# xiph/LPCNet

Hardware: AMD Instinct MI355X
Metric: 16 kHz samples/sec & concurrent real-time streams, 1/2/4/8 MI355X (higher is better)
Workload: dtype f32; 1 GPU; 2048 concurrent streams (each with its own feature file) per GPU x 25 frames (4000 samples) per step, fp32 weights, register-resident block-sparse GRU-A, bit-exact (PARITY) arithmetic; eight streams per CU as two groups of four half a step apart (BASELINE config 2's 1024 streams fill half of these stream slots: `also.config2_1024_streams`); arithmetic=parity, gru_a_blocks=1382, gru_a_densities=0.05,0.05,0.2 (benchmark model), gru_a_items_per_lane=30, streams_per_gpu=2048, streams_per_workgroup=8

## Files before the change

lpcnet_amd/csrc/sample_kernel_x2.hip.h:

```cpp
#pragma once
#include "sample_kernel.hip.h"
#include "tree_stages.h"

namespace lpcn {

#define LPCN_X2_LW 4
#define LPCN_X2_TW 0
#define LPCN_X2_HG 10

struct LdsX2 {
    static constexpr int S = 4;
    static constexpr int HA_STRIDE = 16 * S;
    static constexpr int g_hA    = 0;
    static constexpr int g_hT    = g_hA + 96 * HA_STRIDE + 24 * 16;
    static constexpr int g_prec  = g_hT + NA * S * 4;
    static constexpr int g_hB    = g_prec + NA * S * 4;
    static constexpr int g_idx   = g_hB + S * NB * 4;
    static constexpr int g_thr   = g_idx + S * 16;
    static constexpr int g_mask  = g_thr + S * 32;
    static constexpr int g_lead  = g_mask + S * 64;
    static constexpr int g_flag  = g_lead + S * 32;
    static constexpr int g_condb = g_flag + 16;
    static constexpr int g_lpc   = g_condb + S * RB * 4;
    static constexpr int g_pcm   = g_lpc + S * 64;
    static constexpr int G_SZ    = g_pcm + S * 320;
    static constexpr int pre_ur  = 2 * G_SZ;
    static constexpr int inh     = pre_ur + 2 * NA * S * 4;
    static constexpr int abias   = inh + NA * S * 4;
    static constexpr int tansig  = abias + 2 * RA * 4;
    static constexpr int ulaw    = tansig + 816;
    static constexpr int logit   = ulaw + 1024;
    static constexpr int brec    = logit + 1024;
    static constexpr int bbias   = brec + NB * RB * 4;
    static constexpr int bstart  = bbias + 2 * RB * 4;
    static constexpr int bw      = bstart + 32;
    static constexpr int total(int nb_b) { return bw + (nb_b + 8) * 128; }
    __host__ __device__ static constexpr int ha_off(int p) { return p * HA_STRIDE + (p >> 2) * 16; }
};

typedef float tree_f4 __attribute__((ext_vector_type(4)));
struct TreeRow { tree_f4 w[NB / 4]; float bias, factor; };
template <int STAGE>
__device__ __forceinline__ TreeRow tree_row_load(const LPCN_GLOBAL float *fc_w, const LPCN_GLOBAL float *fc_b, const LPCN_GLOBAL float *fc_f, const int lane, const int prefix)
{
    const int node = lpcn_tree_node(STAGE, lpcn_tree_lane_local(STAGE, lane), prefix), chan = lane & 1;
    const auto *wp = (const LPCN_GLOBAL tree_f4 *)(fc_w + (node * 2 + chan) * NB);
    TreeRow r;
#pragma unroll
    for (int j = 0; j < NB / 4; ++j) r.w[j] = wp[j];
    r.bias = fc_b[chan * 256 + node];
    r.factor = fc_f[chan * 256 + node];
    return r;
}
template <int STAGE>
__device__ __forceinline__ int tree_stage_walk(const TreeRow &r, const float *h_s, const float *thr_s, const float *tansig, const int lane)
{
    const float4 *hp = (const float4 *)h_s;
    float sum = r.bias;
#pragma unroll
    for (int j = 0; j < NB / 4; ++j) {
        const float4 hv = hp[j];
        const tree_f4 wv = r.w[j];
        sum = sum + wv[0] * hv.x;
        sum = sum + wv[1] * hv.y;
        sum = sum + wv[2] * hv.z;
        sum = sum + wv[3] * hv.w;
    }
    const float v = r.factor * lpcn_tanh(sum, tansig);
    const float vo = __builtin_bit_cast(float, __builtin_amdgcn_mov_dpp(__builtin_bit_cast(int, v), 0xB1, 0xf, 0xf, true));
    const float lg = v + vo;
    const unsigned long long m = __ballot(thr_s[lpcn_tree_level(STAGE, lpcn_tree_lane_local(STAGE, lane))] < lg) & lpcn_tree_stage_mask(STAGE);
    return lpcn_tree_stage_walk(m, STAGE == 0 ? LPCN_TREE_TOP : LPCN_TREE_LEVELS - LPCN_TREE_TOP);
}

template <int NW>
__global__ __launch_bounds__(LPCN_WG_THREADS, 2) void sample_kernel_x2(const LpcnSampleArgs *__restrict__ Ap)
{
    using L = LdsX2;
    constexpr int S = 4;
    constexpr int LW = LPCN_X2_LW, TW = LPCN_X2_TW;
    extern __shared__ __attribute__((aligned(16))) unsigned char smem[];
    float *const sm_pre_ur = (float *)(smem + L::pre_ur);
    float *const sm_inh = (float *)(smem + L::inh);
    const float *const sm_abias = (const float *)(smem + L::abias);
    const float *const sm_tansig = (const float *)(smem + L::tansig);
    const float *const sm_ulaw = (const float *)(smem + L::ulaw);
    const float *const sm_logit = (const float *)(smem + L::logit);
    const float *const sm_brec = (const float *)(smem + L::brec);
    const float *const sm_bbias = (const float *)(smem + L::bbias);
    const int *const sm_bstart = (const int *)(smem + L::bstart);

    const int tid0 = threadIdx.x;
    const int n_streams = Ap->n_streams, n_frames = Ap->n_frames, preload = Ap->preload, frame_len = Ap->frame_len;
    const int s0 = blockIdx.x * 2 * S;
    auto stream_of = [&](int gs) __attribute__((always_inline)) { return (s0 + gs < n_streams) ? s0 + gs : n_streams - 1; };
    const int n_valid = (n_streams - s0 < 2 * S) ? n_streams - s0 : 2 * S;
    const size_t nf = (size_t)n_frames;
    auto *const states = as_global_rw(Ap->state);
    const LPCN_GLOBAL float *emb_nat_sig = as_global(Ap->emb_nat_sig), *emb_nat_pred = as_global(Ap->emb_nat_pred), *emb_nat_exc = as_global(Ap->emb_nat_exc);
    asm volatile("" : "+s"(emb_nat_sig), "+s"(emb_nat_pred), "+s"(emb_nat_exc));

    float4 w[NW];
    uint32_t offp[(NW + 1) / 2];
    int row_reg[3];
#define LPCN_ROW(k) (row_reg[k])
    {
        const int lane = tid0 & 63, wave = tid0 >> 6;
        const size_t base = (size_t)wave * NW * 64 + lane;
        const int lane_sel = (lane & 3) * 16;
        const auto *ab = as_global(Ap->a_blk);
        const auto *aw = (const LPCN_GLOBAL float *)as_global(Ap->a_w);
#pragma unroll
        for (int j = 0; j < NW; ++j) {
            const auto *v = aw + (base + (size_t)j * 64) * 4;
            w[j] = make_float4(v[0], v[1], v[2], v[3]);
        }
#pragma unroll
        for (int j = 0; j < NW; j += 2) {
            const int p0 = ab[base + (size_t)j * 64];
            const int p1 = (j + 1 < NW) ? ab[base + (size_t)(j + 1) * 64] : 0;
            offp[j >> 1] = (uint32_t)(L::ha_off(p0) + lane_sel) | ((uint32_t)(L::ha_off(p1) + lane_sel) << 16);
        }
        const auto *ar = as_global(Ap->a_row);
#pragma unroll
        for (int k = 0; k < 3; ++k) row_reg[k] = ar[(wave * 3 + k) * 64 + lane];
    }
    int b1 = __builtin_amdgcn_readfirstlane(as_global(Ap->a_bound)[(tid0 >> 6) * 4 + 1]);
    int b2 = __builtin_amdgcn_readfirstlane(as_global(Ap->a_bound)[(tid0 >> 6) * 4 + 2]);
    int b3 = __builtin_amdgcn_readfirstlane(as_global(Ap->a_bound)[(tid0 >> 6) * 4 + 3]);
    const bool allh0 = __builtin_amdgcn_readfirstlane(as_global(Ap->a_allh)[(tid0 >> 6) * 3]) != 0;
    const LPCN_GLOBAL float *fc_w_s = as_global(Ap->fc_w), *fc_b_s = as_global(Ap->fc_b), *fc_f_s = as_global(Ap->fc_f);
    asm volatile("" : "+s"(fc_w_s), "+s"(fc_b_s), "+s"(fc_f_s));
    const LPCN_GLOBAL float *cond_a_s = as_global(Ap->cond_a);
    asm volatile("" : "+s"(cond_a_s));
    const int has_slot = __builtin_amdgcn_readfirstlane((__ballot(row_reg[0] >= 0) != 0ull ? 1 : 0) | (__ballot(row_reg[1] >= 0) != 0ull ? 2 : 0) |
                                                        (__ballot(row_reg[2] >= 0) != 0ull ? 4 : 0));
    const bool has2 = (has_slot & 4) != 0;
    const int hl = __builtin_amdgcn_readfirstlane(as_global(Ap->a_head)[tid0 >> 6]);
    const bool early_wave = hl > 0;
    const bool plain_start = __builtin_amdgcn_readfirstlane(((early_wave || __ballot(row_reg[0] >= 2 * NA) == 0ull) && __ballot(row_reg[1] >= 2 * NA || row_reg[2] >= 2 * NA) == 0ull) ? 1 : 0) != 0;

    {
        const int tid = tid0;
        stage_tables<L>(smem, Ap, tid, NB * RB);
        stage_grub_weights(smem + L::bw, Ap, tid, true);
        for (int i = tid; i < 2 * S * NA; i += LPCN_WG_THREADS) {
            const int gs = i / NA, n = i % NA, g = gs >> 2, s = gs & 3;
            const float hv0 = states[stream_of(gs)].gru_a[n];
            unsigned char *gb = smem + g * L::G_SZ;
            ((float *)(gb + L::g_hT))[n * S + s] = hv0;
            *(float *)(gb + L::g_hA + L::ha_off(n >> 2) + s * 16 + (n & 3) * 4) = hv0;
        }
        for (int i = tid; i < 2 * S * NB; i += LPCN_WG_THREADS) {
            const int gs = i / NB, g = gs >> 2, s = gs & 3;
            ((float *)(smem + g * L::G_SZ + L::g_hB))[s * NB + i % NB] = states[stream_of(gs)].gru_b[i % NB];
        }
        if (tid < 2 * S) {
            const int g = tid >> 2, s = tid & 3;
            unsigned char *gb = smem + g * L::G_SZ;
            stage_leader_record({(float *)(gb + L::g_lead), (int *)(gb + L::g_idx), nullptr, nullptr}, s, &states[stream_of(tid)]);
        }
        if (tid < 2) { int *fl = (int *)(smem + tid * L::G_SZ + L::g_flag); fl[0] = 0; fl[1] = 0; }
    }
    __syncthreads();

    const bool is_lw = (tid0 >> 6) == LW;
    const bool is_tw_lane = tid0 >= 64 * TW && tid0 < 64 * TW + S;
#define LPCN_LROW ((tid0 & 63) >> 4)
#define LPCN_TAP (tid0 & 15)
    float histP = is_lw ? states[stream_of(S + LPCN_LROW)].last_sig[LPCN_TAP] : 0.f;
    float histQ = is_lw ? states[stream_of(LPCN_LROW)].last_sig[LPCN_TAP] : 0.f;
    bool liveP = false, liveQ = false;
    int live_maskP = 0, live_maskQ = 0;
    int seqP = 0, seqQ = 0;
    int smpP = 0, smpQ = 0, fP = 0, fQ = 0;
    float lpc_tap = 0.f, prod_old = 0.f;

    const int T = n_frames * frame_len;
#if LPCN_ENABLE_PROF
#ifndef LPCN_PROF_MASK
#define LPCN_PROF_MASK 0xFFF
#endif
    unsigned long long *const prof = Ap->prof;
    unsigned long long pt[12] = {0, 0, 0, 0, 0, 0, 0, 0, 0, 0, 0, 0}, tprev = 0;
    const bool profiling = prof != nullptr && blockIdx.x == 0;
#define LPCN_X2_PROF(slot) do { if (((LPCN_PROF_MASK >> (slot)) & 1) && profiling) { const unsigned long long now_ = __builtin_amdgcn_s_memtime(); pt[slot] += now_ - tprev; tprev = now_; } } while (0)
    if (profiling) tprev = __builtin_amdgcn_s_memtime();
#else
#define LPCN_X2_PROF(slot) do { } while (0)
#endif
    for (int h = -1; h <= 2 * T + 1; ++h) {
        const int p = h & 1, q = p ^ 1;
        unsigned char *const gp = smem + p * L::G_SZ, *const gq = smem + q * L::G_SZ;
        const bool p_active = h >= 0 && (h >> 1) < T;
        const bool p_prev = h >= 2;
        const bool q_chain = h >= 1 && ((h - 1) >> 1) < T;
        const bool q_heads = ((h + 1) >> 1) < T;
        const bool new_frame = p_active && smpP == 0;
        const bool more = p_active && smpP != 0;
        float *const hT_p = (float *)(gp + L::g_hT);
        float *const hB_q = (float *)(gq + L::g_hB);
        int *const idx_p = (int *)(gp + L::g_idx);
        float *const lpc_p = (float *)(gp + L::g_lpc);
        short *const pcm_p = (short *)(gp + L::g_pcm);
        const LeaderCells cells_p = {(float *)(gp + L::g_lead), idx_p, (float *)(gp + L::g_thr), pcm_p};
        const uint32_t flag_p = lds_addr(gp + L::g_flag);

        if (more) ++seqP;
        if (p_prev && is_lw) {
            __builtin_amdgcn_s_setprio(3);
            const int smp_done = smpP == 0 ? frame_len - 1 : smpP - 1;
            int t_ = tid0;
            LPCN_REMAT_V(t_);
            const int lrow = (t_ & 63) >> 4, tap = t_ & 15;
            float pcm, deemph;
            int exc;
            draw_sample_walked(cells_p, (const int *)(gp + L::g_mask) + lrow, sm_ulaw, lrow, tap, liveP, smp_done, preload, histP, pcm, deemph, exc);
            if (more) { open_sample<S>(cells_p, tid0, liveP, pcm, tap == 0 ? pcm * lpc_tap : prod_old, exc, false); lds_publish(flag_p, seqP); }
            __builtin_amdgcn_s_setprio(0);
            finish_sample(cells_p, lrow, tap, liveP, smp_done, preload, pcm, deemph);
        }
        if (more && is_tw_lane && liveP) { int t_ = tid0; LPCN_REMAT_V(t_); draw_thresholds(cells_p, sm_logit, t_ - 64 * TW); }

        if (new_frame) {
            int tid = tid0;
            LPCN_REMAT_V(tid);
            const bool lw_ = (tid >> 6) == LW, twl_ = tid >= 64 * TW && tid < 64 * TW + S;
            __syncthreads();
            if (fP > 0) {
                auto *out = as_global_rw(Ap->pcm);
                const size_t pstride = (size_t)Ap->pcm_stride;
                for (int i = tid; i < S * LPCN_FRAME_SIZE; i += LPCN_WG_THREADS) {
                    const int s = i / LPCN_FRAME_SIZE, k = i % LPCN_FRAME_SIZE;
                    if (S * p + s < n_valid && k < frame_len) out[(size_t)(s0 + S * p + s) * pstride + (size_t)(fP - 1) * LPCN_FRAME_SIZE + k] = pcm_p[i];
                }
            }
            __syncthreads();
            {
                const auto *cb = as_global(Ap->cond_b), *lp = as_global(Ap->lpc);
                float *const condb_p = (float *)(gp + L::g_condb);
                if (tid < S * RB) condb_p[tid] = cb[((size_t)stream_of(S * p + tid / RB) * nf + fP) * RB + tid % RB];
                if (tid >= 256 && tid < 256 + S * LPCN_LPC_ORDER) {
                    const int i = tid - 256;
                    lpc_p[i] = lp[((size_t)stream_of(S * p + i / LPCN_LPC_ORDER) * nf + fP) * LPCN_LPC_ORDER + i % LPCN_LPC_ORDER];
                }
                if (lw_ || twl_) {
                    const int lstream = stream_of(S * p + (lw_ ? (tid & 63) >> 4 : tid - 64 * TW));
                    liveP = stream_is_live(Ap, states, lstream, fP);
                }
                if (preload > 0 && tid < S) {
                    const auto *pin = as_global(Ap->pcm) + (size_t)stream_of(S * p + tid) * (size_t)Ap->pcm_stride + (size_t)fP * LPCN_FRAME_SIZE;
                    for (int i = 0; i < preload; ++i) pcm_p[tid * LPCN_FRAME_SIZE + i] = pin[i];
                }
            }
            __syncthreads();
            ++seqP;
            if (lw_) {
                open_sample<S>(cells_p, tid0, liveP, histP, histP * lpc_p[tid & 63], ((const int *)cells_p.lead)[((tid & 63) >> 4) * 8 + 2], true);
                lds_publish(flag_p, seqP);
            }
            if (twl_ && liveP) draw_thresholds(cells_p, sm_logit, tid - 64 * TW);
            __syncthreads();
            int lm = 0;
#pragma unroll
            for (int s = 0; s < S; ++s) lm |= (idx_p[S + s] ? 1 : 0) << s;
            live_maskP = __builtin_amdgcn_readfirstlane(lm);
        }

        LPCN_X2_PROF(0);
        float acc[S] = {};
        constexpr int PF = 2;
        float4 hq[PF + 1] = {};
        const unsigned char *hA_cur = gp + L::g_hA;
        auto fetch_h = [&](const int j) __attribute__((always_inline)) {
            uint32_t pk = offp[j >> 1];
            LPCN_REMAT_V(pk);
            const uint32_t off = (j & 1) ? (pk >> 16) : (pk & 0xFFFFu);
            hq[j % (PF + 1)] = *(const float4 *)(hA_cur + off);
        };
        typedef float negz_t __attribute__((ext_vector_type(4)));
        negz_t negz = {-0.f, -0.f, -0.f, -0.f};
        auto load_negz = [&]() __attribute__((always_inline)) { negz = (negz_t){-0.f, -0.f, -0.f, -0.f}; asm volatile("" : "+v"(negz)); };
        auto mac = [&](const int j) __attribute__((always_inline)) {
            typedef float f4 __attribute__((ext_vector_type(4)));
            typedef float f2 __attribute__((ext_vector_type(2)));
            const float4 hv = hq[j % (PF + 1)];
            const float hk[4] = {hv.x, hv.y, hv.z, hv.w};
            const float wk[4] = {w[j].x, w[j].y, w[j].z, w[j].w};
            f2 a01 = {acc[0], acc[1]}, a23 = {acc[2], acc[3]};
            f4 pv[4];
#pragma unroll
            for (int c = 0; c < 4; ++c) pv[c] = __builtin_amdgcn_mfma_f32_4x4x1f32(hk[c], wk[c], negz, 0, 0, 0);
            __builtin_amdgcn_sched_barrier(0);
#pragma unroll
            for (int c = 0; c < 4; ++c) {
                a01 = a01 + __builtin_shufflevector(pv[c], pv[c], 0, 1);
                a23 = a23 + __builtin_shufflevector(pv[c], pv[c], 2, 3);
            }
            acc[0] = a01[0]; acc[1] = a01[1]; acc[2] = a23[0]; acc[3] = a23[1];
        };
        auto pre_cell = [&](const int r, unsigned char *gb) __attribute__((always_inline)) -> float * {
            return (float *)(r < 2 * NA ? smem + L::pre_ur + r * (S * 4) : gb + L::g_prec + (r - 2 * NA) * (S * 4));
        };

        const int wave = __builtin_amdgcn_readfirstlane(tid0 >> 6);

        constexpr int J0 = NW - LPCN_EARLY_MAX < 0 ? 0 : NW - LPCN_EARLY_MAX;
        constexpr int JM = J0 + LPCN_X2_HG < NW ? J0 + LPCN_X2_HG : NW;
        const bool do_heads = early_wave && q_heads;
        int e0 = NW - hl;
        LPCN_REMAT_S(e0);
        auto head_step = [&](auto self, auto jc, auto jend_c) __attribute__((always_inline)) -> void {
            constexpr int j = decltype(jc)::value, je = decltype(jend_c)::value;
            if constexpr (j < je) {
                if constexpr (j + PF < NW) fetch_h(j + PF);
                if (j >= e0) { asm volatile(""); mac(j); }
                self(self, std::integral_constant<int, j + 1>{}, jend_c);
            }
        };
        const uint32_t p0cnt_p = flag_p + 4;
        constexpr int CW = LPCN_X2_CHAIN_WAVES, P0W = LPCN_X2_P0_FIRST, NP0 = LPCN_WAVES - P0W;
        static_assert(NP0 * 64 * 3 == 2 * NA && CW == S, "three rounds of the row waves' lanes cover GRU-A's update / reset rows");
        const bool p0_wave = p_active && wave >= P0W;
        uint32_t o_sig[S] = {}, o_pred[S] = {}, o_exc[S] = {}, o_cond[S] = {};
        constexpr int P0PERM = 0x3102;
        int i0 = 0;
        float ld[3][4 * S] = {};
        auto p0_open = [&]() __attribute__((always_inline)) {
            int gi[S];
            {
                typedef int i4 __attribute__((ext_vector_type(4)));
                i4 v;
                int f;
                const uint32_t idx_a = lds_addr(idx_p);
                do {
                    asm volatile("ds_read_b32 %0, %2\n\tds_read_b128 %1, %3\n\ts_waitcnt lgkmcnt(0)" : "=&v"(f), "=&v"(v) : "v"(flag_p), "v"(idx_a) : "memory");
                    f = __builtin_amdgcn_readfirstlane(f);
                } while (f != seqP);
#pragma unroll
                for (int s = 0; s < S; ++s) gi[s] = __builtin_amdgcn_readfirstlane(v[s]);
            }
#pragma unroll
            for (int s = 0; s < S; ++s) {
                o_sig[s] = (uint32_t)(gi[s] & 0xFF) * (uint32_t)(RA * 4);
                o_pred[s] = (uint32_t)((gi[s] >> 8) & 0xFF) * (uint32_t)(RA * 4);
                o_exc[s] = ((uint32_t)(gi[s] >> 16) & 0xFFu) * (uint32_t)(RA * 4);
                o_cond[s] = (uint32_t)(((size_t)stream_of(S * p + s) * nf + (size_t)fP) * RA * 4);
            }
            int t_ = tid0;
            LPCN_REMAT_V(t_);
            i0 = (((P0PERM >> (4 * ((t_ >> 6) & 3))) & 3) << 6) | (t_ & 63);
        };
        const bool fifth = ((P0PERM >> (4 * (wave & 3))) & 3) < 2;
        auto issue = [&](const int k, const int buf) __attribute__((always_inline)) {
            const uint32_t rb = (uint32_t)(i0 + 256 * k) * 4u;
#pragma unroll
            for (int s = 0; s < S; ++s) {
                ld[buf][4 * s + 0] = *(const LPCN_GLOBAL float *)((const LPCN_GLOBAL char *)cond_a_s + (o_cond[s] + rb));
                ld[buf][4 * s + 1] = *(const LPCN_GLOBAL float *)((const LPCN_GLOBAL char *)emb_nat_sig + (o_sig[s] + rb));
                ld[buf][4 * s + 2] = *(const LPCN_GLOBAL float *)((const LPCN_GLOBAL char *)emb_nat_pred + (o_pred[s] + rb));
                ld[buf][4 * s + 3] = *(const LPCN_GLOBAL float *)((const LPCN_GLOBAL char *)emb_nat_exc + (o_exc[s] + rb));
            }
        };
        auto reduce = [&](const int k, const int buf) __attribute__((always_inline)) {
            const int r = i0 + 256 * k;
            float g[S];
#pragma unroll
            for (int s = 0; s < S; ++s) g[s] = ((ld[buf][4 * s + 0] + ld[buf][4 * s + 1]) + ld[buf][4 * s + 2]) + ld[buf][4 * s + 3];
            if (k < 3) {
                const int n = r >= NA ? r - NA : r;
                const float2 bd = *(const float2 *)(sm_abias + 2 * r);
                const float4 hv = *(const float4 *)(hT_p + n * S);
                *(float4 *)(sm_pre_ur + r * S) = make_float4((bd.x + bd.y * hv.x) + g[0], (bd.x + bd.y * hv.y) + g[1], (bd.x + bd.y * hv.z) + g[2], (bd.x + bd.y * hv.w) + g[3]);
            } else {
                *(float4 *)(sm_inh + (r - 2 * NA) * S) = make_float4(g[0], g[1], g[2], g[3]);
            }
        };
        if (wave < CW) {
            if (q_chain) {
                __builtin_amdgcn_s_setprio(3);
                const int s = wave;
                int ln_ = tid0;
                LPCN_REMAT_V(ln_);
                ln_ &= 63;
                const int r = ln_ < RB ? ln_ : RB - 1;
                const int g6 = r >> 3, ri = r & 7;
                const float *const condb_q = (const float *)(gq + L::g_condb);
                float zrh = sm_bbias[r] + condb_q[s * RB + r];
                float rec = sm_bbias[RB + r];
#pragma unroll
                for (int j = 0; j < NB; ++j) rec = rec + sm_brec[j * RB + r] * hB_q[s * NB + j];
                uint32_t wp32 = lds_addr(smem + L::bw + (sm_bstart[g6] * 8 + ri) * 16 + ((LPCN_GRUB_SHIFT >> (4 * g6)) & 15) * 128);
                uint32_t hp32 = lds_addr(gq + L::g_hA + s * 16);
                asm volatile(
#include "grub_lds_loop_s4.inc"
                    : [z] "+v"(zrh), [wp] "+v"(wp32), [hp] "+v"(hp32) : : LPCN_GRUB_LDS_CLOBBERS);
                __builtin_amdgcn_s_setprio(0);
                LPCN_X2_PROF(1);
                const TreeRow top = tree_row_load<0>(fc_w_s, fc_b_s, fc_f_s, ln_, 0);
                const int ln = ln_ & 15;
                const float sg = lpcn_sigmoid(zrh + rec, sm_tansig);
                const float r_gate = __builtin_bit_cast(float, __builtin_amdgcn_ds_bpermute((16 + ln) << 2, __builtin_bit_cast(int, sg)));
                const float hc = lpcn_tanh(zrh + rec * r_gate, sm_tansig);
                const float hc_i = __builtin_bit_cast(float, __builtin_amdgcn_ds_bpermute((32 + ln) << 2, __builtin_bit_cast(int, hc)));
                if (ln_ < NB) {
                    const float hold = hB_q[s * NB + ln_];
                    const float hnew = sg * hold + (1.f - sg) * hc_i;
                    if ((live_maskQ >> s) & 1) hB_q[s * NB + ln_] = hnew;
                }
                LPCN_X2_PROF(2);
                const float *const thr_s = (const float *)(gq + L::g_thr) + s * 8;
                int val = tree_stage_walk<0>(top, hB_q + s * NB, thr_s, sm_tansig, ln_);
                const TreeRow sub = tree_row_load<1>(fc_w_s, fc_b_s, fc_f_s, ln_, val);
                val = (val << (LPCN_TREE_LEVELS - LPCN_TREE_TOP)) | tree_stage_walk<1>(sub, hB_q + s * NB, thr_s, sm_tansig, ln_);
                if (ln_ == 0) ((int *)(gq + L::g_mask))[s] = val;
                LPCN_X2_PROF(9);
            }
        } else {
            if (do_heads) {
                hA_cur = gq + L::g_hA;
                load_negz();
                {
                    int r = LPCN_ROW(0);
                    LPCN_REMAT_V(r);
                    r = r < 0 ? 0 : r;
                    const int n = r - 2 * NA;
                    const float bias = sm_abias[2 * r], diag = sm_abias[2 * r + 1];
                    const float *hT_q = (const float *)(gq + L::g_hT);
#pragma unroll
                    for (int s = 0; s < S; ++s) acc[s] = bias + diag * hT_q[n * S + s];
                }
#pragma unroll
                for (int j = 0; j < PF; ++j) if (J0 + j < NW) fetch_h(J0 + j);
                head_step(head_step, std::integral_constant<int, J0>{}, std::integral_constant<int, JM>{});
            }
            LPCN_X2_PROF(3);
            if (p0_wave) {
                p0_open();
                LPCN_X2_PROF(1);
                issue(0, 0); issue(1, 1); issue(2, 2);
                LPCN_X2_PROF(2);
                reduce(0, 0); reduce(1, 1); reduce(2, 2);
                lds_arrive(p0cnt_p);
                issue(3, 0);
                if (fifth) issue(4, 1);
            }
            LPCN_X2_PROF(4);
            if (do_heads) {
                head_step(head_step, std::integral_constant<int, JM>{}, std::integral_constant<int, NW>{});
                int r = LPCN_ROW(0);
                LPCN_REMAT_V(r);
                if (r >= 0) {
                    float *c = pre_cell(r, gq);
#pragma unroll
                    for (int s = 0; s < S; ++s) c[s] = acc[s];
                }
            }
            if (p0_wave) { reduce(3, 0); if (fifth) reduce(4, 1); }
            LPCN_X2_PROF(3);
        }

        if (p_active) {
            hA_cur = gp + L::g_hA;
            load_negz();
            lds_poll_until<false>(p0cnt_p, seqP * NP0);
            LPCN_X2_PROF(11);
            if (plain_start) {
                int r = LPCN_ROW(0);
                LPCN_REMAT_V(r);
                r = r < 0 ? 0 : r;
                const float *c = pre_cell(r, gp);
#pragma unroll
                for (int s = 0; s < S; ++s) acc[s] = c[s];
            } else {
#pragma unroll
            for (int k = 0; k < 3; ++k) {
                int r = LPCN_ROW(k);
                LPCN_REMAT_V(r);
                const bool live_row = r >= 0;
                r = r < 0 ? 0 : r;
                const bool candidate = r >= 2 * NA;
                const int n = candidate ? r - 2 * NA : 0;
                const float bias = sm_abias[2 * r], diag = sm_abias[2 * r + 1];
                float *c = pre_cell(r, gp);
                const bool parked = k == 0 && early_wave;
#pragma unroll
                for (int s = 0; s < S; ++s) {
                    const float bv = bias + diag * hT_p[n * S + s];
                    if (k == 0) acc[s] = (candidate && !parked) ? bv : c[s];
                    else if (candidate && live_row) c[s] = bv;
                }
            }
            }
            auto row_swap = [&](const int k_done, const int k_next) __attribute__((always_inline)) {
                int r = LPCN_ROW(k_done), r2 = LPCN_ROW(k_next);
                LPCN_REMAT_V(r);
                LPCN_REMAT_V(r2);
                if (r >= 0) {
                    float *c = pre_cell(r, gp);
#pragma unroll
                    for (int s = 0; s < S; ++s) c[s] = acc[s];
                }
                r2 = r2 < 0 ? 0 : r2;
                const float *c2 = pre_cell(r2, gp);
#pragma unroll
                for (int s = 0; s < S; ++s) acc[s] = c2[s];
            };
            auto row_store = [&](const int k) __attribute__((always_inline)) {
                int r = LPCN_ROW(k);
                LPCN_REMAT_V(r);
                if (r >= 0) {
                    float *c = pre_cell(r, gp);
#pragma unroll
                    for (int s = 0; s < S; ++s) c[s] = acc[s];
                }
            };
            const int jend = b3;
            LPCN_X2_PROF(4);
#pragma unroll
            for (int j = 0; j < PF && j < NW; ++j) fetch_h(j);
            LPCN_REMAT_S(b1);
            LPCN_REMAT_S(b2);
            LPCN_REMAT_S(b3);
            int nextb = b1;
            LPCN_REMAT_S(nextb);
            auto item = [&](const int j) __attribute__((always_inline)) -> bool {
                if (__builtin_expect(j >= jend, 0)) return false;
                if (j + PF < NW) fetch_h(j + PF);
                if (__builtin_expect(j == nextb, 0)) {
                    if (j == b1) row_swap(0, 1);
                    if (j == b2) row_swap(1, 2);
                    __builtin_amdgcn_s_waitcnt(0xC07F);
                    nextb = b1 > j ? b1 : (b2 > j ? b2 : NW);
                }
                mac(j);
                return true;
            };
            auto run_items = [&](auto self, auto jc) __attribute__((always_inline)) -> void {
                constexpr int j = decltype(jc)::value;
                if constexpr (j < NW) {
                    if (!item(j)) return;
                    self(self, std::integral_constant<int, j + 1>{});
                }
            };
            run_items(run_items, std::integral_constant<int, 0>{});
            LPCN_X2_PROF(5);
            if (b1 >= jend) {
                row_swap(0, 1);
                row_swap(1, 2);
                row_store(2);
            } else if (b2 >= jend) {
                row_swap(1, 2);
                row_store(2);
            } else {
                row_store(2);
            }
            LPCN_X2_PROF(6);
        }
        if (q_chain && is_lw) {
            int t_ = tid0;
            LPCN_REMAT_V(t_);
            lpc_tap = ((const float *)(gq + L::g_lpc))[t_ & 63];
            prod_old = row_shr1(histQ, 0.f) * lpc_tap;
        }
        LPCN_X2_PROF(9);
        __syncthreads();
        LPCN_X2_PROF(7);

        int tid = tid0;
        LPCN_REMAT_V(tid);
        if (p_active) {
            constexpr int NI = NA * S, NQ = NI / LPCN_WG_THREADS;
            const float *const prec_p = (const float *)(gp + L::g_prec);
            float z[NQ], rg[NQ], a[NQ], hold[NQ];
#pragma unroll
            for (int k = 0; k < NQ; ++k) {
                const int i = tid + k * LPCN_WG_THREADS;
                z[k] = sm_pre_ur[i];
                rg[k] = sm_pre_ur[NI + i];
                a[k] = prec_p[i];
                hold[k] = hT_p[i];
            }
#pragma unroll
            for (int k = 0; k < NQ; ++k) { z[k] = lpcn_sigmoid(z[k], sm_tansig); rg[k] = lpcn_sigmoid(rg[k], sm_tansig); }
#pragma unroll
            for (int k = 0; k < NQ; ++k) a[k] = a[k] * rg[k] + sm_inh[tid + k * LPCN_WG_THREADS];
#pragma unroll
            for (int k = 0; k < NQ; ++k) a[k] = lpcn_tanh(a[k], sm_tansig);
            const unsigned ut = (unsigned)tid;
            const bool live_s = ((live_maskP >> (ut & 3u)) & 1) != 0;
            unsigned char *const ha0 = gp + L::g_hA + L::ha_off((int)(ut >> 4)) + (ut & 3u) * 16u + ((ut >> 2) & 3u) * 4u;
            static_assert(L::ha_off(32) == 32 * L::HA_STRIDE + 8 * 16 && LPCN_WG_THREADS == 512 && S == 4, "gate-stage address stride");
#pragma unroll
            for (int k = 0; k < NQ; ++k) {
                const float hnew = z[k] * hold[k] + (1.f - z[k]) * a[k];
                const float hv = live_s ? hnew : hold[k];
                hT_p[tid + k * LPCN_WG_THREADS] = hv;
                *(float *)(ha0 + k * L::ha_off(32)) = hv;
            }
        }
        LPCN_X2_PROF(8);
        __syncthreads();
        LPCN_X2_PROF(10);

        if (p_active) { if (++smpP == frame_len) { smpP = 0; ++fP; } }
        { const float t = histP; histP = histQ; histQ = t; }
        { const bool t = liveP; liveP = liveQ; liveQ = t; }
        { const int t = live_maskP; live_maskP = live_maskQ; live_maskQ = t; }
        { const int t = seqP; seqP = seqQ; seqQ = t; }
        { const int t = smpP; smpP = smpQ; smpQ = t; }
        { const int t = fP; fP = fQ; fQ = t; }
        asm volatile("; LPCN_SAMPLE_LOOP_END" ::: "memory");
        __builtin_amdgcn_sched_barrier(0);
    }

#if LPCN_ENABLE_PROF
    if (profiling && (tid0 & 63) == 0) {
#pragma unroll
        for (int i = 0; i < 12; ++i) prof[(tid0 >> 6) * 12 + i] += pt[i];
    }
#endif
    __syncthreads();
    {
        auto *out = as_global_rw(Ap->pcm);
        const size_t pstride = (size_t)Ap->pcm_stride;
        for (int i = tid0; i < 2 * S * LPCN_FRAME_SIZE; i += LPCN_WG_THREADS) {
            const int gs = i / LPCN_FRAME_SIZE, k = i % LPCN_FRAME_SIZE;
            const short *pb = (const short *)(smem + (gs >> 2) * L::G_SZ + L::g_pcm);
            if (gs < n_valid && k < frame_len) out[(size_t)(s0 + gs) * pstride + (size_t)(n_frames - 1) * LPCN_FRAME_SIZE + k] = pb[(gs & 3) * LPCN_FRAME_SIZE + k];
        }
    }
    {
        const int tid = tid0;
        for (int i = tid; i < 2 * S * NA; i += LPCN_WG_THREADS) {
            const int gs = i / NA, n = i % NA;
            if (gs < n_valid) states[s0 + gs].gru_a[n] = ((const float *)(smem + (gs >> 2) * L::G_SZ + L::g_hT))[n * S + (gs & 3)];
        }
        for (int i = tid; i < 2 * S * NB; i += LPCN_WG_THREADS) {
            const int gs = i / NB;
            if (gs < n_valid) states[s0 + gs].gru_b[i % NB] = ((const float *)(smem + (gs >> 2) * L::G_SZ + L::g_hB))[(gs & 3) * NB + i % NB];
        }
        if (is_lw) {
            if (LPCN_LROW < n_valid) states[s0 + LPCN_LROW].last_sig[LPCN_TAP] = histP;
            if (S + LPCN_LROW < n_valid) states[s0 + S + LPCN_LROW].last_sig[LPCN_TAP] = histQ;
        }
        if (tid < n_valid) {
            auto *st = &states[s0 + tid];
            const unsigned char *gb = smem + (tid >> 2) * L::G_SZ;
            const int *li = (const int *)(gb + L::g_lead) + (tid & 3) * 8;
            const float *lp = (const float *)(gb + L::g_lpc);
#pragma unroll
            for (int j = 0; j < LPCN_LPC_ORDER; ++j) st->lpc[j] = lp[(tid & 3) * LPCN_LPC_ORDER + j];
            st->deemph_mem = ((const float *)li)[1];
            st->last_exc = li[2];
#pragma unroll
            for (int j = 0; j < 4; ++j) st->rng[j] = (uint32_t)li[4 + j];
        }
    }
#undef LPCN_ROW
#undef LPCN_LROW
#undef LPCN_TAP
}

}
```

lpcnet_amd/csrc/tree_stages.h:

```cpp
#pragma once
#include "lpcnet_math.h"

#define LPCN_TREE_LEVELS 8
#define LPCN_TREE_TOP 5

LPCN_HD constexpr int lpcn_tree_stage_nodes(const int stage) { return stage == 0 ? (1 << LPCN_TREE_TOP) - 1 : (1 << (LPCN_TREE_LEVELS - LPCN_TREE_TOP)) - 1; }
LPCN_HD constexpr int lpcn_tree_lane_local(const int stage, const int lane)
{
    const int k = lane >> 1;
    return (k >= 1 && k <= lpcn_tree_stage_nodes(stage)) ? k : 1;
}
LPCN_HD constexpr int lpcn_tree_local_level(const int k) { return k >= 16 ? 4 : k >= 8 ? 3 : k >= 4 ? 2 : k >= 2 ? 1 : 0; }
LPCN_HD constexpr int lpcn_tree_level(const int stage, const int k) { return (stage == 0 ? 0 : LPCN_TREE_TOP) + lpcn_tree_local_level(k); }
LPCN_HD constexpr int lpcn_tree_node(const int stage, const int k, const int prefix)
{
    const int l = lpcn_tree_local_level(k), root = stage == 0 ? 1 : (1 << LPCN_TREE_TOP) | prefix;
    return (root << l) | (k - (1 << l));
}
LPCN_HD constexpr unsigned long long lpcn_tree_stage_mask(const int stage)
{
    return 0x5555555555555555ull & ((1ull << (2 * lpcn_tree_stage_nodes(stage) + 1)) - 1) & ~3ull;
}
LPCN_HD constexpr int lpcn_tree_stage_walk(const unsigned long long ballot, const int levels)
{
    int val = 0;
    for (int b = 0; b < levels; ++b) val = (val << 1) | (int)((ballot >> (2 * ((1 << b) | val))) & 1ull);
    return val;
}
```

Before: 163.4 million samples/s.

## Offload stage-2 tree walk to a separate wave, packing four streams per wave

The second stage of the hierarchical sampling tree walk is taken off the per-stream leader path. A dedicated row wave now evaluates the stage-2 subtrees of all four streams at once, one 16-lane field per stream. The leader publishes each stage-1 prefix tagged with a sequence number in LDS. The stage-2 wave spin-waits on that prefix, interleaving the wait inside its GRU-A item loop a few items before the end, then writes the final sample index. This shortens the serial critical path of the sampling chain, at the cost of an LDS spin-poll, extra registers for the preloaded subtree row, and added work on one row wave.

```diff
diff --git a/lpcnet_amd/csrc/sample_kernel_x2.hip.h b/lpcnet_amd/csrc/sample_kernel_x2.hip.h
--- a/lpcnet_amd/csrc/sample_kernel_x2.hip.h
+++ b/lpcnet_amd/csrc/sample_kernel_x2.hip.h
@@ -6,6 +6,8 @@
 
 #define LPCN_X2_LW 4
 #define LPCN_X2_TW 0
+#define LPCN_X2_S2W 7
+#define LPCN_X2_S2_LEAD 2
 #define LPCN_X2_HG 10
 
 struct LdsX2 {
@@ -18,6 +20,7 @@
     static constexpr int g_idx   = g_hB + S * NB * 4;
     static constexpr int g_thr   = g_idx + S * 16;
     static constexpr int g_mask  = g_thr + S * 32;
+    static constexpr int g_pfx   = g_mask + S * 4;
     static constexpr int g_lead  = g_mask + S * 64;
     static constexpr int g_flag  = g_lead + S * 32;
     static constexpr int g_condb = g_flag + 16;
@@ -40,10 +43,8 @@
 
 typedef float tree_f4 __attribute__((ext_vector_type(4)));
 struct TreeRow { tree_f4 w[NB / 4]; float bias, factor; };
-template <int STAGE>
-__device__ __forceinline__ TreeRow tree_row_load(const LPCN_GLOBAL float *fc_w, const LPCN_GLOBAL float *fc_b, const LPCN_GLOBAL float *fc_f, const int lane, const int prefix)
+__device__ __forceinline__ TreeRow tree_row_load_node(const LPCN_GLOBAL float *fc_w, const LPCN_GLOBAL float *fc_b, const LPCN_GLOBAL float *fc_f, const int node, const int chan)
 {
-    const int node = lpcn_tree_node(STAGE, lpcn_tree_lane_local(STAGE, lane), prefix), chan = lane & 1;
     const auto *wp = (const LPCN_GLOBAL tree_f4 *)(fc_w + (node * 2 + chan) * NB);
     TreeRow r;
 #pragma unroll
@@ -53,7 +54,15 @@
     return r;
 }
 template <int STAGE>
-__device__ __forceinline__ int tree_stage_walk(const TreeRow &r, const float *h_s, const float *thr_s, const float *tansig, const int lane)
+__device__ __forceinline__ TreeRow tree_row_load(const LPCN_GLOBAL float *fc_w, const LPCN_GLOBAL float *fc_b, const LPCN_GLOBAL float *fc_f, const int lane, const int prefix)
+{
+    return tree_row_load_node(fc_w, fc_b, fc_f, lpcn_tree_node(STAGE, lpcn_tree_lane_local(STAGE, lane), prefix), lane & 1);
+}
+__device__ __forceinline__ TreeRow tree_row_load_packed(const LPCN_GLOBAL float *fc_w, const LPCN_GLOBAL float *fc_b, const LPCN_GLOBAL float *fc_f, const int lane, const int prefix)
+{
+    return tree_row_load_node(fc_w, fc_b, fc_f, lpcn_tree_packed_node(lane, prefix), lane & 1);
+}
+__device__ __forceinline__ unsigned long long tree_node_ballot(const TreeRow &r, const float *h_s, const float *thr, const float *tansig)
 {
     const float4 *hp = (const float4 *)h_s;
     float sum = r.bias;
@@ -69,7 +78,12 @@
     const float v = r.factor * lpcn_tanh(sum, tansig);
     const float vo = __builtin_bit_cast(float, __builtin_amdgcn_mov_dpp(__builtin_bit_cast(int, v), 0xB1, 0xf, 0xf, true));
     const float lg = v + vo;
-    const unsigned long long m = __ballot(thr_s[lpcn_tree_level(STAGE, lpcn_tree_lane_local(STAGE, lane))] < lg) & lpcn_tree_stage_mask(STAGE);
+    return __ballot(*thr < lg);
+}
+template <int STAGE>
+__device__ __forceinline__ int tree_stage_walk(const TreeRow &r, const float *h_s, const float *thr_s, const float *tansig, const int lane)
+{
+    const unsigned long long m = tree_node_ballot(r, h_s, thr_s + lpcn_tree_level(STAGE, lpcn_tree_lane_local(STAGE, lane)), tansig) & lpcn_tree_stage_mask(STAGE);
     return lpcn_tree_stage_walk(m, STAGE == 0 ? LPCN_TREE_TOP : LPCN_TREE_LEVELS - LPCN_TREE_TOP);
 }
 
@@ -161,6 +175,7 @@
             stage_leader_record({(float *)(gb + L::g_lead), (int *)(gb + L::g_idx), nullptr, nullptr}, s, &states[stream_of(tid)]);
         }
         if (tid < 2) { int *fl = (int *)(smem + tid * L::G_SZ + L::g_flag); fl[0] = 0; fl[1] = 0; }
+        if (tid < 2 * S) ((int *)(smem + (tid >> 2) * L::G_SZ + L::g_pfx))[tid & 3] = 0;
     }
     __syncthreads();
 
@@ -410,10 +425,8 @@
                 }
                 LPCN_X2_PROF(2);
                 const float *const thr_s = (const float *)(gq + L::g_thr) + s * 8;
-                int val = tree_stage_walk<0>(top, hB_q + s * NB, thr_s, sm_tansig, ln_);
-                const TreeRow sub = tree_row_load<1>(fc_w_s, fc_b_s, fc_f_s, ln_, val);
-                val = (val << (LPCN_TREE_LEVELS - LPCN_TREE_TOP)) | tree_stage_walk<1>(sub, hB_q + s * NB, thr_s, sm_tansig, ln_);
-                if (ln_ == 0) ((int *)(gq + L::g_mask))[s] = val;
+                const int val = tree_stage_walk<0>(top, hB_q + s * NB, thr_s, sm_tansig, ln_);
+                if (ln_ == 0) lds_publish(lds_addr(gq + L::g_pfx) + s * 4, (seqQ << LPCN_TREE_TOP) | val);
                 LPCN_X2_PROF(9);
             }
         } else {
@@ -460,6 +473,23 @@
             LPCN_X2_PROF(3);
         }
 
+        static_assert(LPCN_X2_S2W > LPCN_X2_LW && LPCN_X2_S2W < LPCN_WAVES && LPCN_TREE_FIELDS == S && LPCN_X2_S2_LEAD >= 1, "stage 2 runs on a row wave other than the leader's, one field per stream");
+        const bool s2_wave = q_chain && wave == LPCN_X2_S2W;
+        TreeRow sub = {};
+        int pfx = 0;
+        auto s2_open = [&]() __attribute__((always_inline)) {
+            int t_ = tid0;
+            LPCN_REMAT_V(t_);
+            const uint32_t cell = lds_addr(gq + L::g_pfx) + (uint32_t)lpcn_tree_packed_field(t_ & 63) * 4u;
+            do {
+                asm volatile("ds_read_b32 %0, %1\n\ts_waitcnt lgkmcnt(0)" : "=v"(pfx) : "v"(cell) : "memory");
+            } while (__ballot((pfx >> LPCN_TREE_TOP) != seqQ) != 0ull);
+            pfx &= (1 << LPCN_TREE_TOP) - 1;
+            sub = tree_row_load_packed(fc_w_s, fc_b_s, fc_f_s, t_ & 63, pfx);
+        };
+        const bool s2_in_items = s2_wave && p_active && b3 > 0;
+        if (s2_wave && !s2_in_items) s2_open();
+
         if (p_active) {
             hA_cur = gp + L::g_hA;
             load_negz();
@@ -522,7 +552,9 @@
             LPCN_REMAT_S(b1);
             LPCN_REMAT_S(b2);
             LPCN_REMAT_S(b3);
-            int nextb = b1;
+            int s2_at = s2_in_items ? (jend > LPCN_X2_S2_LEAD ? jend - LPCN_X2_S2_LEAD : 0) : NW + 1;
+            LPCN_REMAT_S(s2_at);
+            int nextb = b1 < s2_at ? b1 : s2_at;
             LPCN_REMAT_S(nextb);
             auto item = [&](const int j) __attribute__((always_inline)) -> bool {
                 if (__builtin_expect(j >= jend, 0)) return false;
@@ -530,8 +562,10 @@
                 if (__builtin_expect(j == nextb, 0)) {
                     if (j == b1) row_swap(0, 1);
                     if (j == b2) row_swap(1, 2);
+                    if (j == s2_at) s2_open();
                     __builtin_amdgcn_s_waitcnt(0xC07F);
                     nextb = b1 > j ? b1 : (b2 > j ? b2 : NW);
+                    if (s2_at > j && s2_at < nextb) nextb = s2_at;
                 }
                 mac(j);
                 return true;
@@ -557,6 +591,17 @@
             }
             LPCN_X2_PROF(6);
         }
+        if (s2_wave) {
+            int t_ = tid0;
+            LPCN_REMAT_V(t_);
+            const int ln = t_ & 63, f = lpcn_tree_packed_field(ln);
+            const unsigned long long m = tree_node_ballot(sub, hB_q + f * NB, (const float *)(gq + L::g_thr) + f * 8 + lpcn_tree_packed_level(ln), sm_tansig) & lpcn_tree_packed_mask();
+            int walks = 0;
+#pragma unroll
+            for (int k = 0; k < S; ++k) walks |= lpcn_tree_packed_walk(m, k) << (8 * k);
+            if ((ln & (LPCN_TREE_FIELD_LANES - 1)) == 0)
+                ((int *)(gq + L::g_mask))[f] = (pfx << (LPCN_TREE_LEVELS - LPCN_TREE_TOP)) | ((walks >> (8 * f)) & ((1 << (LPCN_TREE_LEVELS - LPCN_TREE_TOP)) - 1));
+        }
         if (q_chain && is_lw) {
             int t_ = tid0;
             LPCN_REMAT_V(t_);
diff --git a/lpcnet_amd/csrc/tree_stages.h b/lpcnet_amd/csrc/tree_stages.h
--- a/lpcnet_amd/csrc/tree_stages.h
+++ b/lpcnet_amd/csrc/tree_stages.h
@@ -27,3 +27,21 @@
     for (int b = 0; b < levels; ++b) val = (val << 1) | (int)((ballot >> (2 * ((1 << b) | val))) & 1ull);
     return val;
 }
+
+#define LPCN_TREE_FIELD_LANES 16
+#define LPCN_TREE_FIELDS 4
+LPCN_HD constexpr int lpcn_tree_packed_field(const int lane) { return lane / LPCN_TREE_FIELD_LANES; }
+LPCN_HD constexpr int lpcn_tree_packed_local(const int lane) { return lpcn_tree_lane_local(1, lane % LPCN_TREE_FIELD_LANES); }
+LPCN_HD constexpr int lpcn_tree_packed_level(const int lane) { return lpcn_tree_level(1, lpcn_tree_packed_local(lane)); }
+LPCN_HD constexpr int lpcn_tree_packed_node(const int lane, const int prefix) { return lpcn_tree_node(1, lpcn_tree_packed_local(lane), prefix); }
+LPCN_HD constexpr unsigned long long lpcn_tree_packed_mask()
+{
+    unsigned long long m = 0;
+    for (int f = 0; f < LPCN_TREE_FIELDS; ++f) m |= lpcn_tree_stage_mask(1) << (LPCN_TREE_FIELD_LANES * f);
+    return m;
+}
+LPCN_HD constexpr int lpcn_tree_packed_walk(const unsigned long long ballot, const int field)
+{
+    return lpcn_tree_stage_walk((ballot >> (LPCN_TREE_FIELD_LANES * field)) & ((1ull << LPCN_TREE_FIELD_LANES) - 1), LPCN_TREE_LEVELS - LPCN_TREE_TOP);
+}
+static_assert(2 * lpcn_tree_stage_nodes(1) + 2 <= LPCN_TREE_FIELD_LANES && LPCN_TREE_FIELDS * LPCN_TREE_FIELD_LANES == 64, "a stage-2 subtree fits a 16-lane field");
```

Result: faster. 168.4 million samples/s (median of 6 runs) (+3.1%).
